# mit-han-lab/distrifuser

Hardware: AMD Instinct MI355X
Metric: end-to-end latency (s) per image, SDXL 50-step DDIM (lower is better)
Workload: dtype bf16; 1 GPU; model=sdxl-base (random init), global_batch=1, image=3840x3840, seq_len=230400, scheduler=ddim, steps_per_image=50, parallelism=patch1, mode=corrected_async_gn, cuda_graph=True

## Files before the change

### distrifuser_amd/csrc/bindings.hip

```cpp

#include <torch/extension.h>
#include <ATen/hip/HIPContext.h>
#include <c10/hip/HIPStream.h>

#include <array>

#include "boundary_plan.h"
#include "kernels.h"

namespace {

int dtype_of(const at::Tensor& t) {
    switch (t.scalar_type()) {
        case at::kBFloat16: return DFA_BF16;
        case at::kHalf: return DFA_F16;
        case at::kFloat: return DFA_F32;
        default: TORCH_CHECK(false, "unsupported dtype ", t.scalar_type());
    }
}

bool is_b16(const at::Tensor& t) {
    return t.scalar_type() == at::kBFloat16 || t.scalar_type() == at::kHalf;
}

// ... 312 lines not shown
                                int64_t kv_splits, at::Tensor o_part, at::Tensor lse_part) {
    auto [p, S, o_shape, lse_shape] = split_kv(q, k, v, kv_splits);
    TORCH_CHECK(o_part.is_cuda() && o_part.scalar_type() == at::kFloat && o_part.is_contiguous() &&
                    o_part.sizes() == at::IntArrayRef(o_shape),
                "o_part must be contiguous fp32 [S,B,Lq,H,D] with S = ", S);
    TORCH_CHECK(lse_part.is_cuda() && lse_part.scalar_type() == at::kFloat &&
                    lse_part.is_contiguous() && lse_part.sizes() == at::IntArrayRef(lse_shape),
                "lse_part must be contiguous fp32 [S,B,H,Lq] with S = ", S);
    p.o_part = o_part.data_ptr<float>();
    p.lse = lse_part.data_ptr<float>();
    launch_flash_attention(p, S, dtype_of(q), cur_stream());
    return S;
}

at::Tensor merge_attention_into(const at::Tensor& o_parts, const at::Tensor& lse_parts,
                                at::ScalarType out_dtype,
                                const c10::optional<at::Tensor>& lse_out) {
    TORCH_CHECK(o_parts.is_cuda() && o_parts.dim() == 5 && o_parts.scalar_type() == at::kFloat &&
                    o_parts.is_contiguous(),
                "merge_attention: o_parts must be contiguous fp32 [S,B,Lq,H,D]");
    MergeAttnParams m{};
    m.S = (int)o_parts.size(0);
    m.B = (int)o_parts.size(1);
    m.Lq = o_parts.size(2);
    m.H = (int)o_parts.size(3);
    m.Dh = (int)o_parts.size(4);
    TORCH_CHECK(m.S >= 1 && m.Dh % 8 == 0, "merge_attention: S >= 1 and head_dim % 8 == 0");
    TORCH_CHECK(lse_parts.is_cuda() && lse_parts.scalar_type() == at::kFloat &&
                    lse_parts.is_contiguous() &&
                    lse_parts.sizes() ==
                        (at::IntArrayRef{(long)m.S, (long)m.B, (long)m.H, (long)m.Lq}),
                "merge_attention: lse_parts must be contiguous fp32 [S,B,H,Lq]");
    auto out = at::empty({(long)m.B, (long)m.Lq, (long)m.H, (long)m.Dh},
                         o_parts.options().dtype(out_dtype));
    m.o_parts = o_parts.data_ptr<float>();
    m.lse_parts = lse_parts.data_ptr<float>();
    m.out = out.data_ptr();
    m.out_dtype = dtype_of(out);
    if (lse_out.has_value()) m.lse = lse_out->data_ptr<float>();
    launch_merge_attention(m, cur_stream());
    return out;
}

std::vector<at::Tensor> merge_attention(const at::Tensor& o_parts, const at::Tensor& lse_parts,
                                        bool out_bf16,
                                        const c10::optional<at::ScalarType>& out_dtype) {
    const at::ScalarType dt = out_dtype.value_or(out_bf16 ? at::kBFloat16 : at::kFloat);
    TORCH_CHECK(dt == at::kBFloat16 || dt == at::kHalf || dt == at::kFloat,
                "merge_attention: out_dtype must be bf16, fp16 or fp32");
    TORCH_CHECK(lse_parts.dim() == 4, "merge_attention: lse_parts must be [S,B,H,Lq]");
    auto lse = at::empty({lse_parts.size(1), lse_parts.size(2), lse_parts.size(3)},
                         lse_parts.options());
    auto out = merge_attention_into(o_parts, lse_parts, dt, lse);
    return {out, lse};
}

std::vector<at::Tensor> flash_attention_ext(const at::Tensor& q, const at::Tensor& k,
                                            const at::Tensor& v, int64_t kv_splits,
                                            bool return_lse) {
    auto [p, S, o_shape, lse_shape] = split_kv(q, k, v, kv_splits);
    const auto f32 = q.options().dtype(at::kFloat);
    const long B = p.B, H = p.H, Lq = p.Lq;
    if (S == 1) {
        if (!return_lse) return {flash_plain(p, q)};
        auto o = flash_out(p, q);
        auto lse = at::empty({B, H, Lq}, f32);
        p.lse = lse.data_ptr<float>();
        launch_flash_attention(p, 1, dtype_of(q), cur_stream());
        return {o.permute({0, 2, 1, 3}), lse};
    }
    auto o_part = at::empty(o_shape, f32);
    auto lse_part = at::empty(lse_shape, f32);
    p.o_part = o_part.data_ptr<float>();
    p.lse = lse_part.data_ptr<float>();
    launch_flash_attention(p, S, dtype_of(q), cur_stream());
    if (!return_lse)
        return {merge_attention_into(o_part, lse_part, q.scalar_type(), c10::nullopt)
                    .permute({0, 2, 1, 3})};
    auto lse = at::empty({B, H, Lq}, f32);
    auto o = merge_attention_into(o_part, lse_part, q.scalar_type(), lse);
    return {o.permute({0, 2, 1, 3}), lse};
}

at::Tensor conv3x3(const at::Tensor& x, const at::Tensor& wp,
                   const c10::optional<at::Tensor>& bias, int64_t cout, int64_t stride,
                   const c10::optional<at::Tensor>& top, const c10::optional<at::Tensor>& bot,
                   const c10::optional<at::Tensor>& residual,
                   const c10::optional<at::Tensor>& bias2, int64_t pad_lo) {
    TORCH_CHECK(x.is_cuda() && x.dim() == 4 && is_b16(x),
                "x must be CUDA bf16 or fp16 [B,Cin,H,W]");
    const auto dt = x.scalar_type();
    TORCH_CHECK(x.stride(3) == 1 && x.stride(2) == x.size(3), "x rows must be contiguous");
    TORCH_CHECK(wp.is_cuda() && wp.dim() == 5 && wp.is_contiguous() && wp.size(0) == 9 &&
                wp.size(3) == 64 && wp.size(4) == 8,
                "wp must be packed [9][KS][CT][64][8]");
    TORCH_CHECK(wp.scalar_type() == dt, "conv3x3: wp must have x's dtype (", dt, "), got ",
                wp.scalar_type());
    TORCH_CHECK(stride == 1 || stride == 2);
    const int B = (int)x.size(0), Cin = (int)x.size(1), H = (int)x.size(2), W = (int)x.size(3);
    TORCH_CHECK(pad_lo == 0 || pad_lo == 1, "conv3x3: pad_lo must be 0 or 1, got ", pad_lo);
    if (pad_lo == 0) {
        TORCH_CHECK(stride == 2, "conv3x3: pad_lo=0 needs stride 2, got ", stride);
        TORCH_CHECK(!top.has_value(), "conv3x3: pad_lo=0 takes no top halo row");
        TORCH_CHECK(H >= 2 && W >= 2, "conv3x3: pad_lo=0 needs H, W >= 2, got ", H, "x", W);
    }
    const int Ho = pad_lo ? (H - 1) / (int)stride + 1 : (H - 2) / 2 + 1;
    const int Wo = pad_lo ? (W - 1) / (int)stride + 1 : (W - 2) / 2 + 1;

    Conv3x3Params p{};
    p.x = reinterpret_cast<const uint16_t*>(x.data_ptr());
    p.wp = reinterpret_cast<const uint16_t*>(wp.data_ptr());
    p.B = B;
    p.Cin = Cin;
    p.Cout = (int)cout;
    p.H = H;
    p.W = W;
    p.Ho = Ho;
    p.Wo = Wo;
    p.KS = (int)wp.size(1);
    p.CT = (int)wp.size(2);
    p.pad_lo = (int)pad_lo;
    TORCH_CHECK(p.KS * 16 >= Cin && p.CT * 32 >= cout, "packed weight too small");
    p.x_sb = x.stride(0);
    p.x_sc = x.stride(1);
    if (const char* dbg = getenv("DFA_CONV_DEBUG")) p.debug = atoi(dbg);
    at::Tensor bias_c;
    if (bias.has_value()) {
        bias_c = b16_param(*bias, x, "conv3x3", "bias");
        TORCH_CHECK(bias_c.numel() == cout);
        p.bias = reinterpret_cast<const uint16_t*>(bias_c.data_ptr());
    }
    auto set_halo = [&](const c10::optional<at::Tensor>& h, const uint16_t*& ptr, int64_t& sb,
                        int64_t& sc) {
        if (!h.has_value()) return;
        const at::Tensor& t = *h;
        TORCH_CHECK(t.scalar_type() == dt, "conv3x3: top/bot halo must have x's dtype (", dt,
                    "), got ", t.scalar_type());
        TORCH_CHECK(t.is_cuda() && t.stride(-1) == 1 && t.size(-1) == W && t.size(1) == Cin,
                    "halo must be [B,Cin,(1,)W] with contiguous rows");
        ptr = reinterpret_cast<const uint16_t*>(t.data_ptr());
        sb = t.stride(0);
        sc = t.stride(1);
    };
    set_halo(top, p.top, p.t_sb, p.t_sc);
    set_halo(bot, p.bot, p.b_sb, p.b_sc);
    at::Tensor b2_c;
    if (bias2.has_value()) {
        b2_c = b16_param(*bias2, x, "conv3x3", "bias2");
        TORCH_CHECK(b2_c.numel() == (int64_t)B * cout, "bias2 must be [B, Cout]");
        p.bias2 = reinterpret_cast<const uint16_t*>(b2_c.data_ptr());
    }
    at::Tensor res_c;
    if (residual.has_value()) {
        res_c = residual->contiguous();
        TORCH_CHECK(res_c.scalar_type() == dt, "conv3x3: residual must have x's dtype (", dt,
                    "), got ", res_c.scalar_type());
        TORCH_CHECK(res_c.sizes() == (at::IntArrayRef{(long)B, (long)cout, (long)Ho, (long)Wo}),
                    "residual must be [B,Cout,Ho,Wo]");
        p.residual = reinterpret_cast<const uint16_t*>(res_c.data_ptr());
    }

    auto o = at::empty({(long)B, (long)cout, (long)Ho, (long)Wo}, x.options());
    p.o = reinterpret_cast<uint16_t*>(o.data_ptr());
    launch_conv3x3(p, (int)stride, dtype_of(x), cur_stream());
    return o;
}

std::vector<at::Tensor> dpm_step(const at::Tensor& n, const void* nc, const at::Tensor& xc,
                                 const c10::optional<at::Tensor>& x0_prev, double g, double ca,
                                 double cb, double cc, double cx, double ce,
                                 const MaskBlend* blend) {
    const void* pp = nullptr;
    at::Tensor p;
    if (x0_prev.has_value()) {
        p = x0_prev->contiguous();
        TORCH_CHECK(p.is_cuda() && p.numel() == xc.numel() && p.scalar_type() == at::kFloat,
                    "x0_prev must be the fp32 state from the previous cfg_dpm_step");
        pp = p.data_ptr();
    }
    auto out = at::empty_like(xc);
    auto x0 = at::empty_like(xc, xc.options().dtype(at::kFloat));
    launch_cfg_dpm_step(n.data_ptr(), nc, xc.data_ptr(), pp, out.data_ptr(), x0.data_ptr(),
                        (float)g, (float)ca, (float)cb, (float)cc, (float)cx, (float)ce,
                        xc.numel(), dtype_of(xc), cur_stream(), blend);
    return {out, x0};
}

std::vector<at::Tensor> cfg_dpm_step(const at::Tensor& noise, const at::Tensor& x,
                                     const c10::optional<at::Tensor>& x0_prev, double g,
                                     double ca, double cb, double cc, double cx, double ce) {
    TORCH_CHECK(noise.is_cuda() && noise.size(0) == 2);
    auto n = noise.contiguous();
    auto xc = x.contiguous();
    TORCH_CHECK(xc.numel() * 2 == n.numel());
    const void* nc =
        reinterpret_cast<const char*>(n.data_ptr()) + xc.numel() * n.element_size();
    return dpm_step(n, nc, xc, x0_prev, g, ca, cb, cc, cx, ce, nullptr);
}

std::vector<at::Tensor> masked_dpm_step(const at::Tensor& noise, const at::Tensor& x,
                                        const c10::optional<at::Tensor>& x0_prev,
                                        const at::Tensor& init, const at::Tensor& init_noise,
                                        const at::Tensor& mask, double g, double ca, double cb,
                                        double cc, double cx, double ce, double sa, double sb) {
    auto a = masked_step_args("masked_dpm_step", noise, x, init, init_noise, mask, sa, sb);
    return dpm_step(a.n, a.nc, a.x, x0_prev, g, ca, cb, cc, cx, ce, &a.blend);
}

at::Tensor layer_norm(const at::Tensor& x_, const at::Tensor& w_, const at::Tensor& b_,
                      double eps) {
    TORCH_CHECK(x_.is_cuda() && is_b16(x_), "layer_norm: bf16 or fp16 only");
    auto x = x_.contiguous();
    const int C = (int)x.size(-1);
    TORCH_CHECK(C % 8 == 0 && C <= 2048, "layer_norm kernel: C % 8 == 0 and C <= 2048");
    auto w = b16_param(w_, x, "layer_norm", "weight");
    auto b = b16_param(b_, x, "layer_norm", "bias");
    auto y = at::empty_like(x);
    launch_layer_norm(x.data_ptr(), nullptr, y.data_ptr(), nullptr, w.data_ptr(), b.data_ptr(),
                      (float)eps, x.numel() / C, C, dtype_of(x), cur_stream());
    return y;
}

std::vector<at::Tensor> add_layer_norm(const at::Tensor& x_, const at::Tensor& res_,
                                       const at::Tensor& w_, const at::Tensor& b_, double eps) {
    TORCH_CHECK(x_.is_cuda() && is_b16(x_), "add_layer_norm: bf16 or fp16 only");
    auto x = x_.contiguous();
    auto res = res_.contiguous();
    TORCH_CHECK(res.scalar_type() == x.scalar_type(), "add_layer_norm: res must have x's dtype (",
                x.scalar_type(), "), got ", res.scalar_type());
    TORCH_CHECK(res.sizes() == x.sizes());
    const int C = (int)x.size(-1);
    TORCH_CHECK(C % 8 == 0 && C <= 2048, "add_layer_norm kernel: C % 8 == 0 and C <= 2048");
    auto w = b16_param(w_, x, "add_layer_norm", "weight");
    auto b = b16_param(b_, x, "add_layer_norm", "bias");
    auto y = at::empty_like(x);
    auto sum = at::empty_like(x);
    launch_layer_norm(x.data_ptr(), res.data_ptr(), y.data_ptr(), sum.data_ptr(), w.data_ptr(),
                      b.data_ptr(), (float)eps, x.numel() / C, C, dtype_of(x), cur_stream());
    return {sum, y};
}

at::Tensor vae_attention(const at::Tensor& q, const at::Tensor& k, const at::Tensor& v) {
    TORCH_CHECK(q.is_cuda() && q.dim() == 3 && q.size(-1) == 512 && is_b16(q),
                "vae_attention: bf16 or fp16 [B, L, 512] only");
    TORCH_CHECK(k.scalar_type() == q.scalar_type(), "vae_attention: k must have q's dtype (",
                q.scalar_type(), "), got ", k.scalar_type());
    TORCH_CHECK(v.scalar_type() == q.scalar_type(), "vae_attention: v must have q's dtype (",
                q.scalar_type(), "), got ", v.scalar_type());
    auto qc = q.contiguous(), kc = k.contiguous(), vc = v.contiguous();
    TORCH_CHECK(kc.sizes() == qc.sizes() && vc.sizes() == qc.sizes());
    VaeAttnParams p{};
    p.q = reinterpret_cast<const uint16_t*>(qc.data_ptr());
    p.k = reinterpret_cast<const uint16_t*>(kc.data_ptr());
    p.v = reinterpret_cast<const uint16_t*>(vc.data_ptr());
    p.B = (int)qc.size(0);
    p.L = qc.size(1);
    p.sb = qc.stride(0);
    p.scale = 1.0f / std::sqrt(512.0f);
    auto o = at::empty_like(qc);
    p.o = reinterpret_cast<uint16_t*>(o.data_ptr());
    launch_vae_attention(p, dtype_of(q), cur_stream());
    return o;
}

std::vector<at::Tensor> mfma_probe(const at::Tensor& a, const at::Tensor& b) {
    TORCH_CHECK(a.is_cuda() && a.sizes() == (at::IntArrayRef{64, 8}));
    auto af = a.to(at::kFloat).contiguous(), bf = b.to(at::kFloat).contiguous();
    auto d = at::zeros({64, 4}, af.options());
    launch_mfma_probe(af.data_ptr<float>(), bf.data_ptr<float>(), d.data_ptr<float>(),
                      cur_stream());
    return {d};
}

std::vector<at::Tensor> mfma_probe32(const at::Tensor& a, const at::Tensor& b) {
    TORCH_CHECK(a.is_cuda() && a.sizes() == (at::IntArrayRef{64, 8}));
    auto af = a.to(at::kFloat).contiguous(), bf = b.to(at::kFloat).contiguous();
    auto d = at::zeros({64, 16}, af.options());
    launch_mfma_probe32(af.data_ptr<float>(), bf.data_ptr<float>(), d.data_ptr<float>(),
                        cur_stream());
    return {d};
}
}

PYBIND11_MODULE(TORCH_EXTENSION_NAME, m) {
    m.def("group_norm_stats", &group_norm_stats, "per-group moments [2,N,G,1,1,1]");
    m.def("group_norm_apply", &group_norm_apply,
          "normalize+affine(+SiLU) from given moments; tokens: write [N, HW, C]",
          pybind11::arg("x"), pybind11::arg("mean"), pybind11::arg("meansq"),
          pybind11::arg("weight"), pybind11::arg("bias"), pybind11::arg("eps"),
          pybind11::arg("silu"), pybind11::arg("tokens") = false);
    m.def("group_norm_silu", &group_norm_silu, "fused GroupNorm(+SiLU); tokens: write [N, HW, C]",
          pybind11::arg("x"), pybind11::arg("num_groups"), pybind11::arg("weight"),
          pybind11::arg("bias"), pybind11::arg("eps"), pybind11::arg("silu"),
          pybind11::arg("tokens") = false);
    m.def("tokens_add_nchw", &tokens_add_nchw,
          "y [N, HW, C] + residual [N, C, H, W] -> [N, C, H, W] (transposing residual add)");
    m.def("geglu", &geglu, "a * gelu(gate) over last-dim halves");
    m.def("gn_merge_stats", &gn_merge_stats,
          "merge stale peer GN moments with fresh local ones (one launch)");
    m.def("cfg_affine_step", &cfg_affine_step, "fused CFG combine + affine scheduler update");
    m.def("flash_attention", &flash_attention, "bf16/fp16 flash attention (chunked stale KV)");
    m.def("flash_attention_ext", &flash_attention_ext,
          "flash attention with split-KV and optional log-sum-exp -> [out] or [out, lse]",
          pybind11::arg("q"), pybind11::arg("k"), pybind11::arg("v"),
          pybind11::arg("kv_splits") = 1, pybind11::arg("return_lse") = false);
    m.def("flash_attention_partial", &flash_attention_partial,
          "split-KV partials into caller buffers (o_part fp32 [S,B,Lq,H,D], lse_part [S,B,H,Lq])");
    m.def("merge_attention", &merge_attention,
          "merge fp32 attention partials by their log-sum-exp -> [out, lse]",
          pybind11::arg("o_parts"), pybind11::arg("lse_parts"), pybind11::arg("out_bf16") = true,
          pybind11::arg("out_dtype") = pybind11::none());
    m.def("cfg_dpm_step", &cfg_dpm_step, "fused CFG + DPM-Solver++(2M) update -> (prev, x0)");
    m.def("masked_affine_step", &masked_affine_step,
          "inpaint: (CFG +) affine scheduler update blended with the re-noised init latents");
    m.def("masked_dpm_step", &masked_dpm_step,
          "inpaint: (CFG +) DPM-Solver++(2M) update, prev blended -> (prev, x0)");
    m.def("inpaint_unet_input", &inpaint_unet_input,
          "inpaint U-Net input [copies,9,h,w] = [latents / scale, mask, masked-image latents]");
    m.def("layer_norm", &layer_norm, "bf16/fp16 fused LayerNorm");
    m.def("add_layer_norm", &add_layer_norm, "bf16/fp16 fused residual-add + LayerNorm -> (sum, y)");
    m.def("vae_attention", &vae_attention, "bf16/fp16 single-head d=512 VAE mid attention");
    m.def("conv3x3", &conv3x3,
          "bf16/fp16 implicit-GEMM 3x3 conv, stride 1/2, in-place halo rows; pad_lo=0 "
          "(stride 2) pads bottom/right only",
          pybind11::arg("x"), pybind11::arg("wp"), pybind11::arg("bias"), pybind11::arg("cout"), pybind11::arg("stride"),
          pybind11::arg("top"), pybind11::arg("bot"), pybind11::arg("residual"), pybind11::arg("bias2"),
          pybind11::arg("pad_lo") = 1);
    m.def("mfma_probe", &mfma_probe, "dump mfma_f32_16x16x32_bf16 fragment mapping");
    m.def("mfma_probe32", &mfma_probe32, "dump mfma_f32_32x32x16_bf16 fragment mapping");
}
```

### distrifuser_amd/csrc/conv.hip

```cpp

#include "dispatch.h"

namespace {

typedef int int32x4_ck __attribute__((ext_vector_type(4)));

__device__ int32x4_ck llvm_amdgcn_raw_buffer_load_x4(
    int32x4_ck srsrc, int voffset, int soffset,
    int glc_slc) __asm("llvm.amdgcn.raw.buffer.load.v4i32");

__device__ __forceinline__ int32x4_ck make_srsrc(const void* base, uint32_t bytes) {
    const uint64_t a = (uint64_t)base;
    int32x4_ck r;
    r.x = (int)(uint32_t)a;
    r.y = (int)(uint32_t)(a >> 32);
    r.z = (int)bytes;
    r.w = 0x00020000;
    return r;
}

template <int S_, int YB_, int XW_, int CIN_T_, int NCT_, int PW_>
struct ConvTile {
    static constexpr int S = S_, YB = YB_, XW = XW_, CIN_T = CIN_T_, NCT = NCT_, PW = PW_;
    static constexpr int NW = YB * XW;
    static constexpr int XB = XW * 32 * PW;
};
using ConvWideS1 = ConvTile<1, 8, 1, 16, 4, 2>;
using ConvNarrowS1 = ConvTile<1, 8, 1, 16, 2, 1>;
using ConvS2 = ConvTile<2, 4, 2, 16, 2, 1>;

struct ConvGrid {
    int nxb, nyb, npix, ncb;
    unsigned blocks;
};
template <class T>
__host__ __device__ __forceinline__ ConvGrid conv_grid(const Conv3x3Params& p) {
    ConvGrid g;
    g.nxb = (p.Wo + T::XB - 1) / T::XB;
    g.nyb = (p.Ho + T::YB - 1) / T::YB;
    g.npix = g.nxb * g.nyb * p.B;
    g.ncb = (p.CT + T::NCT - 1) / T::NCT;
    g.blocks = (unsigned)(8 * g.ncb * ((g.npix + 7) / 8));
    return g;
}

template <class T, bool F16, int PL>
__global__ __launch_bounds__(T::NW * WAVE_SIZE) void conv3x3_kernel(Conv3x3Params p) {
    constexpr int S = T::S, YB = T::YB, XW = T::XW, CIN_T = T::CIN_T, NCT = T::NCT, PW = T::PW;
    constexpr int NW = T::NW, XB = T::XB;
    static_assert(PL == 1 || (PL == 0 && S == 2), "pad_lo = 0 is the stride-2 downsample only");
    constexpr int YIN = (YB - 1) * S + 3;
    constexpr int XIN = (XB - 1) * S + 3;
    constexpr int XP = (S == 1) ? XIN : (XB + 1);
    constexpr int KS_T = CIN_T / 16;
    constexpr int ROW_P = CIN_T * 2 + 8;
    constexpr int NFRAG = 9 * KS_T * NCT;
    constexpr int IN_SZ = S * YIN * XP * ROW_P;
    constexpr int W_SZ = NFRAG * WAVE_SIZE * 16;
    __shared__ char in_lds[2 * IN_SZ];
    __shared__ char w_lds[2 * W_SZ];

    const int tid = threadIdx.x;
    const int wave = tid / WAVE_SIZE;
    const int lane = tid % WAVE_SIZE;
    const int lo = lane & 31;
    const int hi = lane >> 5;
    const int wy = wave / XW;
    const int wx = wave % XW;

    const ConvGrid g = conv_grid<T>(p);
    const int nxb = g.nxb, nyb = g.nyb, npix = g.npix, ncb = g.ncb;
    const int D = blockIdx.x;
    const int cb = (D >> 3) % ncb;
    const int pp = (D & 7) + 8 * ((D >> 3) / ncb);
    if (pp >= npix) return;
    const int b = pp / (nxb * nyb);
    const int pt = pp % (nxb * nyb);
    const int xb0 = (pt % nxb) * XB;
    const int yb0 = (pt / nxb) * YB;

    const uint16_t* xin = p.x + (int64_t)b * p.x_sb;
    const uint16_t* top = p.top ? p.top + (int64_t)b * p.t_sb : nullptr;
    const uint16_t* bot = p.bot ? p.bot + (int64_t)b * p.b_sb : nullptr;

    float16v acc[NCT][PW] = {};

    const int n_cin_tiles = (p.KS * 16 + CIN_T - 1) / CIN_T;
    constexpr int WTRIP = (NFRAG + NW - 1) / NW;
    constexpr int CG = CIN_T / 8;
    constexpr int NXW = (XIN - 1 + 7) / 8;
    constexpr int NXS = (NXW + 7) / 8;
    constexpr int NSLAB = YIN * CG * NXS;
    constexpr int STRIP = (NSLAB + NW - 1) / NW;

    const int gr = (lane & 3) | ((lane & 8) >> 1);
    const int gw = ((lane >> 2) & 1) | (((lane >> 4) & 3) << 1);
    const int32x4_ck desc0 = make_srsrc(
        xin, (uint32_t)(((int64_t)(p.Cin - 1) * p.x_sc + (int64_t)p.H * p.W) * 2));
    const uint32_t voff_inc = (uint32_t)(CIN_T * p.x_sc * 2);
    const bool w_vec = (p.W % 8) == 0;
    uint32_t voff[STRIP];
    uint32_t interior_mask = 0, tail_mask = 0, valid_mask = 0;
#pragma unroll
    for (int sit = 0; sit < STRIP; ++sit) {
        const int slab = sit * NW + wave;
        voff[sit] = 0;
        if (NSLAB % NW != 0 && slab >= NSLAB) continue;
        valid_mask |= 1u << sit;
        const int xs = slab % NXS;
        const int cg = (slab / NXS) % CG;
        const int ry = slab / (NXS * CG);
        const int y_in = yb0 * S - PL + ry;
        const int xw = xs * 8 + gw;
        const int x_in0 = xb0 * S + xw * 8;
        if (y_in >= 0 && y_in < p.H) interior_mask |= 1u << sit;
        if (xb0 * S + (xs * 8 + 7) * 8 + 8 > p.W) tail_mask |= 1u << sit;
        voff[sit] = (uint32_t)(((int64_t)(cg * 8 + gr) * p.x_sc +
                                (int64_t)(y_in >= 0 ? y_in : 0) * p.W + x_in0) * 2);
    }

    auto stage_weights = [&](int cint, char* wb) {
        if (p.debug == 3) return;
#pragma unroll
        for (int it = 0; it < WTRIP; ++it) {
            const int frag = it * NW + wave;
            if (NFRAG % NW != 0 && frag >= NFRAG) break;
            const int ct2 = frag % NCT;
            const int ks2 = (frag / NCT) % KS_T;
            const int tap = frag / (NCT * KS_T);
            const int ct = cb * NCT + ct2;
            char* ldst = wb + (int64_t)frag * WAVE_SIZE * 16;
            if (ct < p.CT) {
                const uint16_t* g =
                    p.wp +
                    (((int64_t)(tap * p.KS + cint * KS_T + ks2) * p.CT + ct) * WAVE_SIZE + lane) *
                        8;
                __builtin_amdgcn_global_load_lds(
                    (const __attribute__((address_space(1))) uint32_t*)g,
                    (__attribute__((address_space(3))) uint32_t*)ldst, 16, 0, 0);
            } else {
                *reinterpret_cast<uint4*>(ldst + lane * 16) = uint4{0, 0, 0, 0};
            }
        }
    };
    uint4 iregs[STRIP];
    auto load_input = [&]() {
        if (p.debug == 1) return;
#pragma unroll
        for (int sit = 0; sit < STRIP; ++sit) {
            iregs[sit] = uint4{0, 0, 0, 0};
            if (!((valid_mask >> sit) & 1)) continue;
            if ((interior_mask >> sit) & 1 && w_vec) {
                iregs[sit] = __builtin_bit_cast(
                    uint4, llvm_amdgcn_raw_buffer_load_x4(desc0, (int)voff[sit], 0, 0));
                voff[sit] += voff_inc;
            }
        }
    };
    auto write_input = [&](int cint, char* inb) {
        if (p.debug == 1) return;
        const int cin0 = cint * CIN_T;
#pragma unroll
        for (int sit = 0; sit < STRIP; ++sit) {
            if (!((valid_mask >> sit) & 1)) continue;
            const int slab = sit * NW + wave;
            const int xs = slab % NXS;
            const int cg = (slab / NXS) % CG;
            const int ry = slab / (NXS * CG);
            const int xw = xs * 8 + gw;
            const int x_in0 = xb0 * S + xw * 8;
            uint4 raw = iregs[sit];
            if ((interior_mask >> sit) & 1) {
                if (w_vec) {
                    if ((tail_mask >> sit) & 1) {
                        const int rem = p.W - x_in0;
                        uint32_t* dw = reinterpret_cast<uint32_t*>(&raw);
#pragma unroll
                        for (int d = 0; d < 4; ++d) {
                            const uint32_t m = (rem >= 2 * d + 2)
                                                   ? 0xffffffffu
                                                   : ((rem == 2 * d + 1) ? 0x0000ffffu : 0u);
                            dw[d] &= m;
                        }
                    }
                } else {
                    const int cin = cin0 + cg * 8 + gr;
                    const int y_in = yb0 * S - PL + ry;
                    if (cin < p.Cin) {
                        const uint16_t* rp = xin + (int64_t)cin * p.x_sc + (int64_t)y_in * p.W;
                        uint16_t vals[8];
#pragma unroll
                        for (int jj = 0; jj < 8; ++jj)
                            vals[jj] = (x_in0 + jj < p.W) ? rp[x_in0 + jj] : (uint16_t)0;
                        raw = *reinterpret_cast<const uint4*>(vals);
                    }
                }
            } else {
                const int y_in = yb0 * S - PL + ry;
                const uint16_t* src = nullptr;
                int64_t sc = 0;
                if (y_in == -1 && top) {
                    src = top;
                    sc = p.t_sc;
                } else if (y_in == p.H && bot) {
                    src = bot;
                    sc = p.b_sc;
                }
                const int cin = cin0 + cg * 8 + gr;
                if (src && cin < p.Cin) {
                    const uint16_t* rp = src + (int64_t)cin * sc;
                    uint16_t vals[8];
#pragma unroll
                    for (int jj = 0; jj < 8; ++jj)
                        vals[jj] = (x_in0 + jj < p.W) ? rp[x_in0 + jj] : (uint16_t)0;
                    raw = *reinterpret_cast<const uint4*>(vals);
                }
            }
            const uint4 tr = transpose8x8_b16(raw, lane);
            const int xi = 1 + xw * 8 + gr;
            if (xi < XIN) {
                const int plane = (S == 1) ? 0 : (xi & 1);
                const int row = (S == 1) ? xi : (xi >> 1);
                char* dst = &inb[((plane * YIN + ry) * XP + row) * ROW_P + cg * 16];
                *reinterpret_cast<uint2*>(dst) = uint2{tr.x, tr.y};
                *reinterpret_cast<uint2*>(dst + 8) = uint2{tr.z, tr.w};
            }
        }
        constexpr int XI_COL = PL ? 0 : XIN;
        for (int c = tid; c < YIN * CIN_T; c += NW * WAVE_SIZE) {
            const int ci = c % CIN_T;
            const int ry = c / CIN_T;
            const int y_in = yb0 * S - PL + ry;
            const int x_in = xb0 * S - 1 + XI_COL;
            const int cin = cin0 + ci;
            uint16_t val = 0;
            if (x_in >= 0 && (PL || x_in < p.W) && cin < p.Cin) {
                if (y_in >= 0 && y_in < p.H)
                    val = xin[(int64_t)cin * p.x_sc + (int64_t)y_in * p.W + x_in];
                else if (y_in == -1 && top)
                    val = top[(int64_t)cin * p.t_sc + x_in];
                else if (y_in == p.H && bot)
                    val = bot[(int64_t)cin * p.b_sc + x_in];
            }
            constexpr int CPLANE = (S == 1) ? 0 : (XI_COL & 1);
            constexpr int CROW = (S == 1) ? XI_COL : (XI_COL >> 1);
            *reinterpret_cast<uint16_t*>(
                &inb[((CPLANE * YIN + ry) * XP + CROW) * ROW_P + ci * 2]) = val;
        }
    };
    auto compute_tile = [&](char* inb, char* wb) {
        if (p.debug != 2) {
#pragma unroll
            for (int tap = 0; tap < 9; ++tap) {
                const int dy = tap / 3;
                const int dx = tap % 3;
                const int ry = wy * S + dy;
#pragma unroll
                for (int ks2 = 0; ks2 < KS_T; ++ks2) {
                    short8 bfrag[PW];
#pragma unroll
                    for (int px = 0; px < PW; ++px) {
                        const int xi = ((wx * PW + px) * 32 + lo) * S + dx + (1 - PL);
                        const int plane = (S == 1) ? 0 : (xi & 1);
                        const int row = (S == 1) ? xi : (xi >> 1);
                        bfrag[px] = lds_frag_b64x2(&inb[((plane * YIN + ry) * XP + row) * ROW_P +
                                                        (ks2 * 16 + hi * 8) * 2]);
                    }
#pragma unroll
                    for (int ct2 = 0; ct2 < NCT; ++ct2) {
                        const short8 afrag = *reinterpret_cast<const short8*>(
                            &wb[(((tap * KS_T + ks2) * NCT + ct2) * WAVE_SIZE + lane) * 16]);
#pragma unroll
                        for (int px = 0; px < PW; ++px)
                            acc[ct2][px] =
                                mfma_32x32x16<F16>(afrag, bfrag[px], acc[ct2][px]);
                    }
                }
            }
        }
    };

    if (n_cin_tiles > 0) {
        stage_weights(0, w_lds);
        load_input();
        write_input(0, in_lds);
    }
    for (int cint = 0; cint < n_cin_tiles; ++cint) {
        char* inb = in_lds + (cint & 1) * IN_SZ;
        char* wb = w_lds + (cint & 1) * W_SZ;
        __syncthreads();
        const bool more = cint + 1 < n_cin_tiles;
        if (more) {
            stage_weights(cint + 1, w_lds + ((cint + 1) & 1) * W_SZ);
            load_input();
        }
        compute_tile(inb, wb);
        if (more) write_input(cint + 1, in_lds + ((cint + 1) & 1) * IN_SZ);
    }


    const int y = yb0 + wy;
    if (y >= p.Ho) return;
#pragma unroll
    for (int px = 0; px < PW; ++px) {
        const int x = xb0 + (wx * PW + px) * 32 + lo;
        if (x >= p.Wo) continue;
        const int64_t pix_off = (int64_t)b * p.Cout * p.Ho * p.Wo + (int64_t)y * p.Wo + x;
        uint16_t* obase = p.o + pix_off;
        const uint16_t* rbase = p.residual ? p.residual + pix_off : nullptr;
#pragma unroll
        for (int ct2 = 0; ct2 < NCT; ++ct2) {
            const int ct = cb * NCT + ct2;
            if (ct >= p.CT) break;
#pragma unroll
            for (int r = 0; r < 16; ++r) {
                const int cout = ct * 32 + mfma32_row(r, hi);
                if (cout < p.Cout) {
                    float v = acc[ct2][px][r];
                    if (p.bias) v += b16_to_f32<F16>(p.bias[cout]);
                    if (p.bias2) v += b16_to_f32<F16>(p.bias2[b * p.Cout + cout]);
                    if (rbase) v += b16_to_f32<F16>(rbase[(int64_t)cout * p.Ho * p.Wo]);
                    obase[(int64_t)cout * p.Ho * p.Wo] = f32_to_b16<F16>(v);
                }
            }
        }
    }
}

template <class T, bool F16, int PL = 1>
void launch_tile(const Conv3x3Params& p, hipStream_t stream) {
    conv3x3_kernel<T, F16, PL>
        <<<dim3(conv_grid<T>(p).blocks), dim3(T::NW * WAVE_SIZE), 0, stream>>>(p);
}

}

void launch_conv3x3(const Conv3x3Params& p, int stride, int dtype, hipStream_t stream) {
    dispatch_f16(dtype, [&]<bool F16>(std::bool_constant<F16>) {
        if (stride != 1) {
            if (p.pad_lo == 0)
                launch_tile<ConvS2, F16, 0>(p, stream);
            else
                launch_tile<ConvS2, F16>(p, stream);
        } else if (p.Wo <= 128) {
            launch_tile<ConvNarrowS1, F16>(p, stream);
        } else {
            launch_tile<ConvWideS1, F16>(p, stream);
        }
    });
}
```

### distrifuser_amd/csrc/kernels.h

```cpp
#pragma once

#include <hip/hip_runtime.h>
#include <cstdint>

enum DfaDtype : int { DFA_BF16 = 0, DFA_F16 = 1, DFA_F32 = 2 };

int gn_stats_chunks(int64_t group_len, int n_groups_total, int dtype);
void launch_gn_stats_partial(const void* x, float* ws, float* partial, int64_t group_len,
                             int n_groups_total, int dtype, hipStream_t stream);
void launch_gn_finalize(const float* partial, void* out, float inv_count,
                        int n_groups_total, int dtype, hipStream_t stream);
void launch_gn_apply(const void* x, void* y, const float* mean, const float* meansq,
                     const void* weight, const void* bias, float eps, int64_t hw,
                     int C, int G, int N, bool silu, int dtype, hipStream_t stream);

void launch_gn_apply_tokens(const void* x, void* y, const float* mean, const float* meansq,
                            const void* weight, const void* bias, float eps, int64_t hw,
                            int C, int G, int N, bool silu, int dtype, hipStream_t stream);

void launch_tokens_add_nchw(const void* y, const void* residual, void* out, int64_t hw, int C,
                            int N, int64_t res_stride_n, int64_t res_stride_c, int dtype,
                            hipStream_t stream);

void launch_gn_merge_stats(void* buffer, int64_t row_stride, int64_t slot_off,
                           int n_peers, int own, const void* fresh, float* out,
                           int ng, bool corrected, int dtype, hipStream_t stream);

void launch_geglu(const void* in, void* out, int64_t rows, int64_t inner, int dtype,
                  hipStream_t stream);

struct MaskBlend {
    const float* init;
    const float* init_noise;
    const float* mask;
    float sa, sb;
    int64_t hw;
};

void launch_cfg_affine_step(const void* noise_u, const void* noise_c, const void* x, void* out,
                            float g, float ca, float cb, int64_t total, int dtype,
                            hipStream_t stream, const MaskBlend* blend = nullptr);

void launch_inpaint_unet_input(const void* latents, const void* mask, const void* masked,
                               void* out, float scale, int64_t hw, int copies, int dtype,
                               hipStream_t stream);

struct Conv3x3Params {
    const uint16_t* x;
    const uint16_t* top;
    const uint16_t* bot;
    const uint16_t* wp;
    const uint16_t* bias;
    const uint16_t* residual;
    const uint16_t* bias2;
    uint16_t* o;
    int B, Cin, Cout, H, W, Ho, Wo;
    int KS, CT;
    int debug;
    int pad_lo;
    int64_t x_sb, x_sc;
    int64_t t_sb, t_sc;
    int64_t b_sb, b_sc;
};
void launch_conv3x3(const Conv3x3Params& p, int stride, int dtype, hipStream_t stream);

void launch_cfg_dpm_step(const void* nu, const void* nc, const void* x, const void* x0_prev,
                         void* out, void* x0_out, float g, float ca, float cb, float cc,
                         float cx, float ce, int64_t total, int dtype, hipStream_t stream,
                         const MaskBlend* blend = nullptr);

void launch_layer_norm(const void* x, const void* res, void* y, void* sum_out,
                       const void* w, const void* b, float eps, int64_t rows, int C,
                       int dtype, hipStream_t stream);

struct VaeAttnParams {
    const uint16_t* q;
    const uint16_t* k;
    const uint16_t* v;
    uint16_t* o;
    int B;
    int64_t L, sb;
    float scale;
};
void launch_vae_attention(const VaeAttnParams& p, int dtype, hipStream_t stream);

struct FlashAttnParams {
    const uint16_t* q;
    const uint16_t* k;
    const uint16_t* v;
    uint16_t* o;
    int B, H;
    int Dh;
    int64_t Lq, NC, LC;
    int64_t q_sb, q_sh, q_sl;
    int64_t k_sb, k_sh, k_sc, k_sl;
    int64_t v_sb, v_sh, v_sc, v_sl;
    float scale;
};

struct FlashAttnLseParams : FlashAttnParams {
    float* lse;
    float* o_part;
};
int flash_attention_num_splits(int64_t lkv, int splits);
void launch_flash_attention(const FlashAttnLseParams& p, int splits, int dtype,
                            hipStream_t stream);

void launch_mfma_probe(const float* a, const float* b, float* d, hipStream_t stream);
void launch_mfma_probe32(const float* a, const float* b, float* d, hipStream_t stream);

struct MergeAttnParams {
    const float* o_parts;
    const float* lse_parts;
    void* out;
    float* lse;
    int S, B, H, Dh;
    int64_t Lq;
    int out_dtype;
};
void launch_merge_attention(const MergeAttnParams& p, hipStream_t stream);
```

### distrifuser_amd/models/resnet.py

```python

from __future__ import annotations

import torch
import torch.distributed as dist
import torch.nn.functional as F
from torch import nn

from ..ops import NativeConv2d
from .layers import LayerFactory


class ResnetBlock2D(nn.Module):

    def __init__(
        self,
        in_channels: int,
        out_channels: int,
        temb_channels: int,
        *,
        factory: LayerFactory,
        groups: int = 32,
        eps: float = 1e-5,
    ):
        super().__init__()
        self.in_channels = in_channels
        self.out_channels = out_channels
        state = factory.state
        n = state.config.n_device_per_batch
        self.tp_pair = (
            factory.parallelism == "tensor"
            and n > 1
            and out_channels % n == 0
            and groups % n == 0
        )
        self.state = state

        self.norm1 = factory.group_norm(groups, in_channels, eps=eps, fuse_silu=True)
        if self.tp_pair:
            rank = state.config.split_idx()
            self.c_local = out_channels // n
            self.c_start = rank * self.c_local
            self.conv1 = NativeConv2d(in_channels, self.c_local, 3, padding=1, bias=True)
            self.time_emb_proj = nn.Linear(temb_channels, self.c_local)
            self.norm2 = nn.GroupNorm(groups // n, self.c_local, eps=eps)
            self.conv2 = NativeConv2d(self.c_local, out_channels, 3, padding=1, bias=False)
            self.conv2_bias = nn.Parameter(torch.zeros(out_channels))
        else:
            self.conv1 = factory.conv2d(in_channels, out_channels, 3, 1, 1)
            self.time_emb_proj = nn.Linear(temb_channels, out_channels)
            self.norm2 = factory.group_norm(groups, out_channels, eps=eps, fuse_silu=True)
            self.conv2 = factory.conv2d(out_channels, out_channels, 3, 1, 1)
        if in_channels != out_channels:
            self.conv_shortcut = NativeConv2d(in_channels, out_channels, 1)
        else:
            self.conv_shortcut = None

    def copy_from_full_tp(self, sd: dict, prefix: str) -> None:
        assert self.tp_pair
        s, e = self.c_start, self.c_start + self.c_local
        self.conv1.weight.data.copy_(sd[f"{prefix}conv1.weight"][s:e])
        self.conv1.bias.data.copy_(sd[f"{prefix}conv1.bias"][s:e])
        self.time_emb_proj.weight.data.copy_(sd[f"{prefix}time_emb_proj.weight"][s:e])
        self.time_emb_proj.bias.data.copy_(sd[f"{prefix}time_emb_proj.bias"][s:e])
        self.norm2.weight.data.copy_(sd[f"{prefix}norm2.weight"][s:e])
        self.norm2.bias.data.copy_(sd[f"{prefix}norm2.bias"][s:e])
        self.conv2.weight.data.copy_(sd[f"{prefix}conv2.weight"][:, s:e])
        self.conv2_bias.data.copy_(sd[f"{prefix}conv2.bias"])

    def forward(self, x: torch.Tensor, temb: torch.Tensor) -> torch.Tensor:
        import os
        t2 = self.time_emb_proj(F.silu(temb))
        if os.environ.get("DFA_NO_TEMB_FUSE", "0") == "1":
            h = self.conv1(self.norm1(x)) + t2[:, :, None, None]
        else:
            h = self.conv1(self.norm1(x), bias2=t2)
        if self.tp_pair:
            h = F.silu(self.norm2(h))
            h = self.conv2(h)
            if dist.is_initialized():
                dist.all_reduce(h, op=dist.ReduceOp.SUM, group=self.state.config.batch_group)
            h = h + self.conv2_bias.view(1, -1, 1, 1)
        else:
            res = self.conv_shortcut(x) if self.conv_shortcut is not None else x
            return self.conv2(self.norm2(h), residual=res)
        if self.conv_shortcut is not None:
            x = self.conv_shortcut(x)
        return x + h


class Downsample2D(nn.Module):
    def __init__(self, channels: int, *, factory: LayerFactory):
        super().__init__()
        self.conv = factory.conv2d(channels, channels, 3, stride=2, padding=1, tp_shard=True)

    def forward(self, x: torch.Tensor) -> torch.Tensor:
        return self.conv(x)


class Upsample2D(nn.Module):
    def __init__(self, channels: int, *, factory: LayerFactory):
        super().__init__()
        self.conv = factory.conv2d(channels, channels, 3, stride=1, padding=1, tp_shard=True)

    def forward(self, x: torch.Tensor) -> torch.Tensor:
        x = F.interpolate(x, scale_factor=2.0, mode="nearest")
        return self.conv(x)
```

### distrifuser_amd/ops/__init__.py

```python

from .conv import NativeConv2d, conv3x3_halo, pack_conv3x3_weight
from .dispatch import (
    add_layer_norm,
    attention_kv_splits,
    flash_attention,
    flash_attention_chunked,
    geglu,
    group_norm_apply,
    group_norm_silu,
    group_norm_stats,
    hip_ext,
    hip_ext_available,
    inpaint_unet_input,
    layer_norm,
    masked_affine_step,
    masked_dpm_step,
    merge_attention,
    tokens_add_nchw,
    use_hip,
    vae_attention,
)
from .norm import PlainGroupNorm

__all__ = [
    "NativeConv2d",
    "PlainGroupNorm",
    "add_layer_norm",
    "attention_kv_splits",
    "layer_norm",
    "conv3x3_halo",
    "flash_attention",
    "flash_attention_chunked",
    "geglu",
    "group_norm_apply",
    "group_norm_silu",
    "group_norm_stats",
    "hip_ext",
    "hip_ext_available",
    "inpaint_unet_input",
    "masked_affine_step",
    "masked_dpm_step",
    "merge_attention",
    "pack_conv3x3_weight",
    "tokens_add_nchw",
    "use_hip",
    "vae_attention",
]
```

### distrifuser_amd/ops/conv.py

```python

from __future__ import annotations

import torch
from torch import nn

from . import eager
from .dispatch import use_hip, hip_ext


_CONV_DTYPES = (torch.bfloat16, torch.float16)


def pack_conv3x3_weight(weight: torch.Tensor, dtype: torch.dtype | None = None) -> torch.Tensor:
    dtype = torch.bfloat16 if dtype is None else dtype
    if dtype not in _CONV_DTYPES:
        raise ValueError(f"pack_conv3x3_weight: dtype must be bf16 or fp16, got {dtype}")
    cout, cin, kh, kw = weight.shape
    assert kh == 3 and kw == 3, "pack_conv3x3_weight is 3x3 only"
    cin_p = (cin + 63) // 64 * 64
    cout_p = (cout + 31) // 32 * 32
    wp = weight.new_zeros(cout_p, cin_p, 9, dtype=torch.float32)
    wp[:cout, :cin] = weight.reshape(cout, cin, 9).float()
    ks, ct = cin_p // 16, cout_p // 32
    wp = wp.permute(2, 1, 0)
    wp = wp.reshape(9, ks, 2, 8, ct, 32)
    wp = wp.permute(0, 1, 4, 2, 5, 3)
    return wp.reshape(9, ks, ct, 64, 8).contiguous().to(dtype)


def _hip_conv_ok(x: torch.Tensor, stride: int) -> bool:
    return (
        x.dtype in _CONV_DTYPES
        and stride in (1, 2)
        and x.stride(-1) == 1
        and x.stride(-2) == x.shape[-1]
    )


def conv3x3_halo(x, weight, bias, stride=1, top=None, bot=None, packed=None, residual=None,
                 bias2=None, pad_lo=1):
    import os
    if residual is not None and os.environ.get("DFA_CONV_RESID", "0") != "1":
        out = conv3x3_halo(x, weight, bias, stride, top, bot, packed=packed, bias2=bias2,
                           pad_lo=pad_lo)
        return out + residual
    if use_hip(x) and packed is not None and _hip_conv_ok(x, stride):
        cout = weight.shape[0]
        t = top.reshape(top.shape[0], top.shape[1], -1) if top is not None else None
        b = bot.reshape(bot.shape[0], bot.shape[1], -1) if bot is not None else None
        if (t is None or t.stride(-1) == 1) and (b is None or b.stride(-1) == 1):
            return hip_ext().conv3x3(x, packed, bias, cout, stride, t, b, residual, bias2,
                                     pad_lo)
    out = eager.conv3x3_halo(x, weight, bias, stride, top, bot, pad_lo)
    if bias2 is not None:
        out = out + bias2.to(out.dtype)[:, :, None, None]
    return out if residual is None else out + residual


class NativeConv2d(nn.Conv2d):

    def __init__(self, *args, asym_pad: bool = False, **kwargs):
        super().__init__(*args, **kwargs)
        if asym_pad and not (self.kernel_size == (3, 3) and self.stride == (2, 2)
                             and self.padding == (0, 0)):
            raise ValueError("asym_pad needs a 3x3 conv with stride 2 and padding 0")
        self.asym_pad = asym_pad
        self._wp = None
        self._wp_key = None

    def _native_eligible(self, x: torch.Tensor) -> bool:
        return (
            x.is_cuda
            and self.kernel_size == (3, 3)
            and self.padding == ((0, 0) if self.asym_pad else (1, 1))
            and self.stride[0] == self.stride[1]
            and self.stride[0] in (1, 2)
            and self.dilation == (1, 1)
            and self.groups == 1
            and x.dtype in _CONV_DTYPES
        )

    def packed_weight(self) -> torch.Tensor:
        w = self.weight
        key = (w._version, w.data_ptr(), w.dtype, w.device)
        if self._wp is None or self._wp_key != key:
            with torch.no_grad():
                self._wp = pack_conv3x3_weight(
                    w.detach(), torch.float16 if w.dtype == torch.float16 else None)
            self._wp_key = key
        return self._wp

    def forward(self, x: torch.Tensor, top=None, bot=None, residual=None,
                bias2=None) -> torch.Tensor:
        if self._native_eligible(x):
            if not _hip_conv_ok(x, self.stride[0]):
                x = x.contiguous()
            return conv3x3_halo(
                x, self.weight, self.bias, self.stride[0], top, bot,
                packed=self.packed_weight(), residual=residual, bias2=bias2,
                pad_lo=0 if self.asym_pad else 1,
            )
        if (
            x.is_cuda
            and self.kernel_size == (1, 1)
            and self.stride == (1, 1)
            and self.groups == 1
            and top is None
            and bot is None
        ):
            b, c, h, w = x.shape
            out = torch.matmul(self.weight.view(self.out_channels, c),
                               x.reshape(b, c, h * w))
            if self.bias is not None:
                out = out + self.bias.view(1, -1, 1)
            return out.view(b, self.out_channels, h, w)
        if self.asym_pad:
            out = eager.conv3x3_halo(x, self.weight, self.bias, 2, top, bot, pad_lo=0)
        elif top is None and bot is None:
            out = super().forward(x)
        else:
            out = eager.conv3x3_halo(x, self.weight, self.bias, self.stride[0], top, bot)
        if bias2 is not None:
            out = out + bias2.to(out.dtype)[:, :, None, None]
        return out if residual is None else out + residual
```

Measured before the change: 27.78 s/image.

## Fuse nearest 2x upsample into 3x3 conv via parity-collapsed weights

Adds a conv3x3_up2 kernel path that computes the 3x3 convolution of the 2x nearest-upsampled input straight from the source tensor. The 3x3 weights are collapsed per output parity into four 2x2 kernels (16 taps), so each source pixel feeds four accumulators. This skips materialising the 4x larger upsampled tensor and cuts MACs from 9 to 4 per output pixel. It uses a new tile config with four accumulators per wave. The Upsample2D module routes to it when the conv runs on the whole image (not patch-parallel), and an env var can disable it.

Result: no change. 27.58 s/image, median of 6 (-0.7%).

```diff
diff --git a/distrifuser_amd/csrc/bindings.hip b/distrifuser_amd/csrc/bindings.hip
--- a/distrifuser_amd/csrc/bindings.hip
+++ b/distrifuser_amd/csrc/bindings.hip
@@ -418,18 +418,19 @@
     return {o.permute({0, 2, 1, 3}), lse};
 }
 
-at::Tensor conv3x3(const at::Tensor& x, const at::Tensor& wp,
-                   const c10::optional<at::Tensor>& bias, int64_t cout, int64_t stride,
-                   const c10::optional<at::Tensor>& top, const c10::optional<at::Tensor>& bot,
-                   const c10::optional<at::Tensor>& residual,
-                   const c10::optional<at::Tensor>& bias2, int64_t pad_lo) {
+at::Tensor conv3x3_impl(const at::Tensor& x, const at::Tensor& wp,
+                        const c10::optional<at::Tensor>& bias, int64_t cout, int64_t stride,
+                        const c10::optional<at::Tensor>& top,
+                        const c10::optional<at::Tensor>& bot,
+                        const c10::optional<at::Tensor>& residual,
+                        const c10::optional<at::Tensor>& bias2, int64_t pad_lo, bool up2) {
     TORCH_CHECK(x.is_cuda() && x.dim() == 4 && is_b16(x),
                 "x must be CUDA bf16 or fp16 [B,Cin,H,W]");
     const auto dt = x.scalar_type();
     TORCH_CHECK(x.stride(3) == 1 && x.stride(2) == x.size(3), "x rows must be contiguous");
-    TORCH_CHECK(wp.is_cuda() && wp.dim() == 5 && wp.is_contiguous() && wp.size(0) == 9 &&
-                wp.size(3) == 64 && wp.size(4) == 8,
-                "wp must be packed [9][KS][CT][64][8]");
+    TORCH_CHECK(wp.is_cuda() && wp.dim() == 5 && wp.is_contiguous() &&
+                wp.size(0) == (up2 ? 16 : 9) && wp.size(3) == 64 && wp.size(4) == 8,
+                "wp must be packed [", up2 ? 16 : 9, "][KS][CT][64][8]");
     TORCH_CHECK(wp.scalar_type() == dt, "conv3x3: wp must have x's dtype (", dt, "), got ",
                 wp.scalar_type());
     TORCH_CHECK(stride == 1 || stride == 2);
@@ -440,8 +441,10 @@
         TORCH_CHECK(!top.has_value(), "conv3x3: pad_lo=0 takes no top halo row");
         TORCH_CHECK(H >= 2 && W >= 2, "conv3x3: pad_lo=0 needs H, W >= 2, got ", H, "x", W);
     }
-    const int Ho = pad_lo ? (H - 1) / (int)stride + 1 : (H - 2) / 2 + 1;
-    const int Wo = pad_lo ? (W - 1) / (int)stride + 1 : (W - 2) / 2 + 1;
+    TORCH_CHECK(!up2 || (stride == 1 && pad_lo == 1 && H >= 1 && W >= 1),
+                "conv3x3_up2: stride 1, pad 1 and a non-empty image");
+    const int Ho = up2 ? 2 * H : pad_lo ? (H - 1) / (int)stride + 1 : (H - 2) / 2 + 1;
+    const int Wo = up2 ? 2 * W : pad_lo ? (W - 1) / (int)stride + 1 : (W - 2) / 2 + 1;
 
     Conv3x3Params p{};
     p.x = reinterpret_cast<const uint16_t*>(x.data_ptr());
@@ -456,6 +459,7 @@
     p.KS = (int)wp.size(1);
     p.CT = (int)wp.size(2);
     p.pad_lo = (int)pad_lo;
+    p.up2 = up2;
     TORCH_CHECK(p.KS * 16 >= Cin && p.CT * 32 >= cout, "packed weight too small");
     p.x_sb = x.stride(0);
     p.x_sc = x.stride(1);
@@ -500,6 +504,20 @@
     p.o = reinterpret_cast<uint16_t*>(o.data_ptr());
     launch_conv3x3(p, (int)stride, dtype_of(x), cur_stream());
     return o;
+}
+
+at::Tensor conv3x3(const at::Tensor& x, const at::Tensor& wp,
+                   const c10::optional<at::Tensor>& bias, int64_t cout, int64_t stride,
+                   const c10::optional<at::Tensor>& top, const c10::optional<at::Tensor>& bot,
+                   const c10::optional<at::Tensor>& residual,
+                   const c10::optional<at::Tensor>& bias2, int64_t pad_lo) {
+    return conv3x3_impl(x, wp, bias, cout, stride, top, bot, residual, bias2, pad_lo, false);
+}
+
+at::Tensor conv3x3_up2(const at::Tensor& x, const at::Tensor& wp,
+                       const c10::optional<at::Tensor>& bias, int64_t cout) {
+    return conv3x3_impl(x, wp, bias, cout, 1, c10::nullopt, c10::nullopt, c10::nullopt,
+                        c10::nullopt, 1, true);
 }
 
 std::vector<at::Tensor> dpm_step(const at::Tensor& n, const void* nc, const at::Tensor& xc,
@@ -662,6 +680,10 @@
           pybind11::arg("x"), pybind11::arg("wp"), pybind11::arg("bias"), pybind11::arg("cout"), pybind11::arg("stride"),
           pybind11::arg("top"), pybind11::arg("bot"), pybind11::arg("residual"), pybind11::arg("bias2"),
           pybind11::arg("pad_lo") = 1);
+    m.def("conv3x3_up2", &conv3x3_up2,
+          "bf16/fp16 conv3x3 (pad 1) of the 2x nearest upsample of x, from the source tensor and "
+          "the parity-collapsed pack [16][KS][CT][64][8]",
+          pybind11::arg("x"), pybind11::arg("wp"), pybind11::arg("bias"), pybind11::arg("cout"));
     m.def("mfma_probe", &mfma_probe, "dump mfma_f32_16x16x32_bf16 fragment mapping");
     m.def("mfma_probe32", &mfma_probe32, "dump mfma_f32_32x32x16_bf16 fragment mapping");
 }
diff --git a/distrifuser_amd/csrc/conv.hip b/distrifuser_amd/csrc/conv.hip
--- a/distrifuser_amd/csrc/conv.hip
+++ b/distrifuser_amd/csrc/conv.hip
@@ -19,15 +19,19 @@
     return r;
 }
 
-template <int S_, int YB_, int XW_, int CIN_T_, int NCT_, int PW_>
+template <int S_, int YB_, int XW_, int CIN_T_, int NCT_, int PW_, bool UP_ = false>
 struct ConvTile {
     static constexpr int S = S_, YB = YB_, XW = XW_, CIN_T = CIN_T_, NCT = NCT_, PW = PW_;
+    static constexpr bool UP = UP_;
     static constexpr int NW = YB * XW;
     static constexpr int XB = XW * 32 * PW;
+    static constexpr int NTAP = UP ? 16 : 9;
+    static constexpr int NACC = UP ? 4 : PW;
 };
 using ConvWideS1 = ConvTile<1, 8, 1, 16, 4, 2>;
 using ConvNarrowS1 = ConvTile<1, 8, 1, 16, 2, 1>;
 using ConvS2 = ConvTile<2, 4, 2, 16, 2, 1>;
+using ConvUp2 = ConvTile<1, 8, 1, 16, 2, 1, true>;
 
 struct ConvGrid {
     int nxb, nyb, npix, ncb;
@@ -36,8 +40,8 @@
 template <class T>
 __host__ __device__ __forceinline__ ConvGrid conv_grid(const Conv3x3Params& p) {
     ConvGrid g;
-    g.nxb = (p.Wo + T::XB - 1) / T::XB;
-    g.nyb = (p.Ho + T::YB - 1) / T::YB;
+    g.nxb = ((T::UP ? p.W : p.Wo) + T::XB - 1) / T::XB;
+    g.nyb = ((T::UP ? p.H : p.Ho) + T::YB - 1) / T::YB;
     g.npix = g.nxb * g.nyb * p.B;
     g.ncb = (p.CT + T::NCT - 1) / T::NCT;
     g.blocks = (unsigned)(8 * g.ncb * ((g.npix + 7) / 8));
@@ -48,13 +52,17 @@
 __global__ __launch_bounds__(T::NW * WAVE_SIZE) void conv3x3_kernel(Conv3x3Params p) {
     constexpr int S = T::S, YB = T::YB, XW = T::XW, CIN_T = T::CIN_T, NCT = T::NCT, PW = T::PW;
     constexpr int NW = T::NW, XB = T::XB;
+    constexpr bool UP = T::UP;
+    constexpr int NTAP = T::NTAP;
+    static_assert(!UP || (S == 1 && PL == 1 && PW == 1 && XW == 1),
+                  "the upsample mode is a stride-1, pad-1 tile of one 32-x subtile per wave");
     static_assert(PL == 1 || (PL == 0 && S == 2), "pad_lo = 0 is the stride-2 downsample only");
     constexpr int YIN = (YB - 1) * S + 3;
     constexpr int XIN = (XB - 1) * S + 3;
     constexpr int XP = (S == 1) ? XIN : (XB + 1);
     constexpr int KS_T = CIN_T / 16;
     constexpr int ROW_P = CIN_T * 2 + 8;
-    constexpr int NFRAG = 9 * KS_T * NCT;
+    constexpr int NFRAG = NTAP * KS_T * NCT;
     constexpr int IN_SZ = S * YIN * XP * ROW_P;
     constexpr int W_SZ = NFRAG * WAVE_SIZE * 16;
     __shared__ char in_lds[2 * IN_SZ];
@@ -83,7 +91,7 @@
     const uint16_t* top = p.top ? p.top + (int64_t)b * p.t_sb : nullptr;
     const uint16_t* bot = p.bot ? p.bot + (int64_t)b * p.b_sb : nullptr;
 
-    float16v acc[NCT][PW] = {};
+    float16v acc[NCT][T::NACC] = {};
 
     const int n_cin_tiles = (p.KS * 16 + CIN_T - 1) / CIN_T;
     constexpr int WTRIP = (NFRAG + NW - 1) / NW;
@@ -249,7 +257,32 @@
         }
     };
     auto compute_tile = [&](char* inb, char* wb) {
-        if (p.debug != 2) {
+        if constexpr (UP) {
+            if (p.debug == 2) return;
+#pragma unroll
+            for (int sh = 0; sh < 9; ++sh) {
+                const int dy = sh / 3;
+                const int dx = sh % 3;
+#pragma unroll
+                for (int ks2 = 0; ks2 < KS_T; ++ks2) {
+                    const short8 bfrag = lds_frag_b64x2(
+                        &inb[((wy + dy) * XP + lo + dx) * ROW_P + (ks2 * 16 + hi * 8) * 2]);
+#pragma unroll
+                    for (int par = 0; par < 4; ++par) {
+                        const int a = dy - (par >> 1);
+                        const int bb = dx - (par & 1);
+                        if (a < 0 || a > 1 || bb < 0 || bb > 1) continue;
+                        const int tap = par * 4 + a * 2 + bb;
+#pragma unroll
+                        for (int ct2 = 0; ct2 < NCT; ++ct2) {
+                            const short8 afrag = *reinterpret_cast<const short8*>(
+                                &wb[(((tap * KS_T + ks2) * NCT + ct2) * WAVE_SIZE + lane) * 16]);
+                            acc[ct2][par] = mfma_32x32x16<F16>(afrag, bfrag, acc[ct2][par]);
+                        }
+                    }
+                }
+            }
+        } else if (p.debug != 2) {
 #pragma unroll
             for (int tap = 0; tap < 9; ++tap) {
                 const int dy = tap / 3;
@@ -300,6 +333,28 @@
 
 
     const int y = yb0 + wy;
+    if constexpr (UP) {
+        const int x = xb0 + lo;
+        if (y >= p.H || x >= p.W) return;
+        const int64_t plane = (int64_t)p.Ho * p.Wo;
+        uint16_t* obase = p.o + (int64_t)b * p.Cout * plane + (int64_t)(2 * y) * p.Wo + 2 * x;
+#pragma unroll
+        for (int ct2 = 0; ct2 < NCT; ++ct2) {
+            const int ct = cb * NCT + ct2;
+            if (ct >= p.CT) break;
+#pragma unroll
+            for (int r = 0; r < 16; ++r) {
+                const int cout = ct * 32 + mfma32_row(r, hi);
+                if (cout >= p.Cout) continue;
+                const float bv = p.bias ? b16_to_f32<F16>(p.bias[cout]) : 0.f;
+#pragma unroll
+                for (int py = 0; py < 2; ++py)
+                    *reinterpret_cast<uint32_t*>(obase + (int64_t)cout * plane + py * p.Wo) =
+                        pack2_b16<F16>(acc[ct2][py * 2][r] + bv, acc[ct2][py * 2 + 1][r] + bv);
+            }
+        }
+        return;
+    }
     if (y >= p.Ho) return;
 #pragma unroll
     for (int px = 0; px < PW; ++px) {
@@ -337,7 +392,9 @@
 
 void launch_conv3x3(const Conv3x3Params& p, int stride, int dtype, hipStream_t stream) {
     dispatch_f16(dtype, [&]<bool F16>(std::bool_constant<F16>) {
-        if (stride != 1) {
+        if (p.up2) {
+            launch_tile<ConvUp2, F16>(p, stream);
+        } else if (stride != 1) {
             if (p.pad_lo == 0)
                 launch_tile<ConvS2, F16, 0>(p, stream);
             else
diff --git a/distrifuser_amd/csrc/kernels.h b/distrifuser_amd/csrc/kernels.h
--- a/distrifuser_amd/csrc/kernels.h
+++ b/distrifuser_amd/csrc/kernels.h
@@ -58,6 +58,7 @@
     int KS, CT;
     int debug;
     int pad_lo;
+    int up2;
     int64_t x_sb, x_sc;
     int64_t t_sb, t_sc;
     int64_t b_sb, b_sc;
diff --git a/distrifuser_amd/models/resnet.py b/distrifuser_amd/models/resnet.py
--- a/distrifuser_amd/models/resnet.py
+++ b/distrifuser_amd/models/resnet.py
@@ -1,5 +1,7 @@
 
 from __future__ import annotations
+
+import os
 
 import torch
 import torch.distributed as dist
@@ -7,6 +9,7 @@
 from torch import nn
 
 from ..ops import NativeConv2d
+from ..parallel.patch_ops import PatchConv2d, _is_patch_parallel
 from .layers import LayerFactory
 
 
@@ -101,7 +104,18 @@
     def __init__(self, channels: int, *, factory: LayerFactory):
         super().__init__()
         self.conv = factory.conv2d(channels, channels, 3, stride=1, padding=1, tp_shard=True)
+        self.fuse = os.environ.get("DFA_NO_UPSAMPLE_FUSE", "0") != "1"
+
+    def _whole_image_conv(self) -> NativeConv2d | None:
+        conv = self.conv
+        if isinstance(conv, PatchConv2d):
+            conv = None if _is_patch_parallel(conv.state) else conv.conv
+        return conv if isinstance(conv, NativeConv2d) else None
 
     def forward(self, x: torch.Tensor) -> torch.Tensor:
+        if self.fuse:
+            conv = self._whole_image_conv()
+            if conv is not None and conv.up2_eligible(x):
+                return conv.forward_up2(x)
         x = F.interpolate(x, scale_factor=2.0, mode="nearest")
         return self.conv(x)
diff --git a/distrifuser_amd/ops/__init__.py b/distrifuser_amd/ops/__init__.py
--- a/distrifuser_amd/ops/__init__.py
+++ b/distrifuser_amd/ops/__init__.py
@@ -1,5 +1,10 @@
 
-from .conv import NativeConv2d, conv3x3_halo, pack_conv3x3_weight
+from .conv import (
+    NativeConv2d,
+    conv3x3_halo,
+    pack_conv3x3_up2_weight,
+    pack_conv3x3_weight,
+)
 from .dispatch import (
     add_layer_norm,
     attention_kv_splits,
@@ -41,6 +46,7 @@
     "masked_affine_step",
     "masked_dpm_step",
     "merge_attention",
+    "pack_conv3x3_up2_weight",
     "pack_conv3x3_weight",
     "tokens_add_nchw",
     "use_hip",
diff --git a/distrifuser_amd/ops/conv.py b/distrifuser_amd/ops/conv.py
--- a/distrifuser_amd/ops/conv.py
+++ b/distrifuser_amd/ops/conv.py
@@ -2,6 +2,7 @@
 from __future__ import annotations
 
 import torch
+import torch.nn.functional as F
 from torch import nn
 
 from . import eager
@@ -26,6 +27,40 @@
     wp = wp.reshape(9, ks, 2, 8, ct, 32)
     wp = wp.permute(0, 1, 4, 2, 5, 3)
     return wp.reshape(9, ks, ct, 64, 8).contiguous().to(dtype)
+
+
+_UP2_TAPS = (((0,), (1, 2)), ((0, 1), (2,)))
+
+
+def collapse_conv3x3_up2_weight(weight: torch.Tensor) -> torch.Tensor:
+    w = weight.float()
+    cout, cin = w.shape[:2]
+    wp = w.new_zeros(2, 2, 2, 2, cout, cin)
+    for py in range(2):
+        for px in range(2):
+            for a in range(2):
+                for b in range(2):
+                    for ky in _UP2_TAPS[py][a]:
+                        for kx in _UP2_TAPS[px][b]:
+                            wp[py, px, a, b] += w[:, :, ky, kx]
+    return wp
+
+
+def pack_conv3x3_up2_weight(weight: torch.Tensor, dtype: torch.dtype | None = None) -> torch.Tensor:
+    dtype = torch.bfloat16 if dtype is None else dtype
+    if dtype not in _CONV_DTYPES:
+        raise ValueError(f"pack_conv3x3_up2_weight: dtype must be bf16 or fp16, got {dtype}")
+    cout, cin, kh, kw = weight.shape
+    assert kh == 3 and kw == 3, "pack_conv3x3_up2_weight is 3x3 only"
+    cin_p = (cin + 63) // 64 * 64
+    cout_p = (cout + 31) // 32 * 32
+    wp = weight.new_zeros(16, cout_p, cin_p, dtype=torch.float32)
+    wp[:, :cout, :cin] = collapse_conv3x3_up2_weight(weight).reshape(16, cout, cin)
+    ks, ct = cin_p // 16, cout_p // 32
+    wp = wp.permute(0, 2, 1)
+    wp = wp.reshape(16, ks, 2, 8, ct, 32)
+    wp = wp.permute(0, 1, 4, 2, 5, 3)
+    return wp.reshape(16, ks, ct, 64, 8).contiguous().to(dtype)
 
 
 def _hip_conv_ok(x: torch.Tensor, stride: int) -> bool:
@@ -67,6 +102,8 @@
         self.asym_pad = asym_pad
         self._wp = None
         self._wp_key = None
+        self._wp_up2 = None
+        self._wp_up2_key = None
 
     def _native_eligible(self, x: torch.Tensor) -> bool:
         return (
@@ -89,6 +126,32 @@
                     w.detach(), torch.float16 if w.dtype == torch.float16 else None)
             self._wp_key = key
         return self._wp
+
+    def packed_up2_weight(self) -> torch.Tensor:
+        w = self.weight
+        key = (w._version, w.data_ptr(), w.dtype, w.device)
+        if self._wp_up2 is None or self._wp_up2_key != key:
+            with torch.no_grad():
+                self._wp_up2 = pack_conv3x3_up2_weight(
+                    w.detach(), torch.float16 if w.dtype == torch.float16 else None)
+            self._wp_up2_key = key
+        return self._wp_up2
+
+    def up2_eligible(self, x: torch.Tensor) -> bool:
+        return (
+            self._native_eligible(x)
+            and use_hip(x)
+            and not self.asym_pad
+            and self.stride == (1, 1)
+            and x.dim() == 4
+            and x.dtype == self.weight.dtype
+            and _hip_conv_ok(x, 1)
+        )
+
+    def forward_up2(self, x: torch.Tensor) -> torch.Tensor:
+        if not self.up2_eligible(x):
+            return self(F.interpolate(x, scale_factor=2.0, mode="nearest"))
+        return hip_ext().conv3x3_up2(x, self.packed_up2_weight(), self.bias, self.out_channels)
 
     def forward(self, x: torch.Tensor, top=None, bot=None, residual=None,
                 bias2=None) -> torch.Tensor:
```
